# tatary/ramses

Measured on AMD Instinct MI355X. Metric: cell-updates/s (Godunov sweep), uniform Sedov3D, higher is better.
Workload: dtype f64

## Files before the change

ramses_amd/csrc/hydro_sweep.hip:

```cpp
#include <hip/hip_runtime.h>

#include <type_traits>

#include "difmag_core.hpp"
#include "hydro_core.hpp"
#include "sweep_args.hpp"

namespace ramses_amd {

#ifdef RAMSES_AMD_FAST
#define SWEEP_NS fastmode
#else
#define SWEEP_NS strictmode
#endif

namespace SWEEP_NS {

constexpr int BX = 64;
#ifndef TILE_SWEEP_BY
#define TILE_SWEEP_BY 12
#endif

template <int BY, int NV>
struct Plane {
  double v[NV][BY][BX];
};

template <int ST, int BY, int NV, bool MASK, bool GRAV, int NX = 0, bool DUTY = false, bool R3 = false, int DPN = 0>
struct Lds {
  static constexpr int NF = NV + NX;
  static constexpr int RING = (ST == 3 || R3) ? 3 : 2;
#ifndef SWEEP_PARK_PLAIN
#ifdef RAMSES_AMD_FAST
#define SWEEP_PARK_PLAIN 1
#else
#define SWEEP_PARK_PLAIN 0
#endif
#endif
  static constexpr bool PARK = MASK || ((GRAV || SWEEP_PARK_PLAIN) && BY == 12);
  static constexpr int MR = PARK ? BY - 2 : BY;
  static constexpr int M0 = PARK ? 1 : 0;
  static constexpr size_t q_off = 0;
  static constexpr size_t m_off = q_off + RING * sizeof(Plane<BY, NV>);
  static constexpr size_t park_off = m_off + 2 * sizeof(Plane<MR, NF>);
  static constexpr size_t duty_off = park_off + (PARK ? sizeof(double) * 2 * NF * (BY - 4) * BX : 0);
  static constexpr size_t mask_off = duty_off + (DUTY ? sizeof(double) * 2 * NF * BX : 0);
  static constexpr size_t sloc_off = mask_off + (MASK ? 3 * BY * BX : 0);
  static constexpr size_t dpark_off = sloc_off + (MASK ? 4 * BY * BX : 0);
  static constexpr size_t bytes = dpark_off + sizeof(double) * DPN * (BY - 4) * BX;
};
template <int RS, int NV>
constexpr int dif_parked() { return (NV == 5 && RS == RIEMANN_EXACT) ? 2 * NV + 2 : ((NV == 6) ? NV + 2 : 0); }

__device__ __forceinline__ double wave_shr1(double v) {
  int lo = __double2loint(v), hi = __double2hiint(v);
  lo = __builtin_amdgcn_update_dpp(lo, lo, 0x138, 0xf, 0xf, false);
  hi = __builtin_amdgcn_update_dpp(hi, hi, 0x138, 0xf, 0xf, false);
  return __hiloint2double(hi, lo);
}
template <bool TIED = false>
__device__ __forceinline__ double wave_shl1(double v) {
  int lo = __double2loint(v), hi = __double2hiint(v);
  lo = TIED ? __builtin_amdgcn_update_dpp(lo, lo, 0x130, 0xf, 0xf, false) : __builtin_amdgcn_update_dpp(0, lo, 0x130, 0xf, 0xf, true);
  hi = TIED ? __builtin_amdgcn_update_dpp(hi, hi, 0x130, 0xf, 0xf, false) : __builtin_amdgcn_update_dpp(0, hi, 0x130, 0xf, 0xf, true);
  return __hiloint2double(hi, lo);
}

enum { ROLE_HALO = 0, ROLE_LOW = 1, ROLE_HIGH = 2, ROLE_FULL = 3, ROLE_HALO_HI = 4, ROLE_FULL_LO = 5 };

#ifndef SWEEP_YDUTY
#define SWEEP_YDUTY 0
#endif
template <int ST, int RS, int BY, bool GRAV, int SCHEME, int NV, bool MASK, int NE = 0, bool PFIX = false>
constexpr bool y_duty() {
  return SWEEP_YDUTY && SWEEP_PARK_PLAIN && RS == RIEMANN_LLF && BY == 12 && ST != 3 && !GRAV && SCHEME == 0 && NV == 5 && !MASK && NE == 0 && !PFIX;
}
template <int BY, bool DUTY>
constexpr int yflux_wave(int f) { return !DUTY ? f : (f == 2 ? 0 : (f == BY - 2 ? BY - 1 : f)); }

#ifndef SWEEP_TRIM
#ifdef RAMSES_AMD_FAST
#define SWEEP_TRIM 1
#else
#define SWEEP_TRIM 0
#endif
#endif

#ifndef SWEEP_CYCLE_PROBE
#define SWEEP_CYCLE_PROBE 0
#endif
#if SWEEP_CYCLE_PROBE
constexpr int PROBE_BLOCKS = 8192, PROBE_ROWS = 12, PROBE_WORDS = 6;
static __device__ unsigned long long sweep_cycle_probe[PROBE_BLOCKS][PROBE_ROWS][PROBE_WORDS];
#endif

typedef unsigned int v2u32 __attribute__((ext_vector_type(2)));
constexpr unsigned BUF_RANGE = 0x7fffffffu;
constexpr unsigned BUF_OOB = 0xffffffffu;
#ifndef SWEEP_STORE_AUX
#define SWEEP_STORE_AUX 0
#endif
__device__ __forceinline__ double plane_load(const double *var_base, unsigned plane_bytes, unsigned off) {
  __amdgpu_buffer_rsrc_t r = __builtin_amdgcn_make_buffer_rsrc(const_cast<double *>(var_base), 0, BUF_RANGE, 0x00020000);
  return __builtin_bit_cast(double, __builtin_amdgcn_raw_buffer_load_b64(r, off, plane_bytes, 0));
}
__device__ __forceinline__ void plane_store(double *var_base, unsigned plane_bytes, unsigned off, double x) {
  __amdgpu_buffer_rsrc_t r = __builtin_amdgcn_make_buffer_rsrc(var_base, 0, BUF_RANGE, 0x00020000);
  __builtin_amdgcn_raw_buffer_store_b64(__builtin_bit_cast(v2u32, x), r, off, plane_bytes, SWEEP_STORE_AUX);
}

__device__ __forceinline__ int wave_shr1_i(int v) { return __builtin_amdgcn_update_dpp(v, v, 0x138, 0xf, 0xf, false); }
__device__ __forceinline__ int wave_shl1_i(int v) { return __builtin_amdgcn_update_dpp(0, v, 0x130, 0xf, 0xf, true); }
__device__ __forceinline__ int stat_load(const unsigned char *base, unsigned ncell, unsigned lane_cell, unsigned plane_cell) {
  __amdgpu_buffer_rsrc_t r = __builtin_amdgcn_make_buffer_rsrc(const_cast<unsigned char *>(base), 0, ncell, 0x00020000);
  return (int)__builtin_amdgcn_raw_buffer_load_b8(r, lane_cell, plane_cell, 0);
}
__device__ __forceinline__ int dir_load(const int *base, unsigned plane_ints, unsigned col) {
  __amdgpu_buffer_rsrc_t r = __builtin_amdgcn_make_buffer_rsrc(const_cast<int *>(base), 0, BUF_RANGE, 0x00020000);
  return (int)__builtin_amdgcn_raw_buffer_load_b32(r, col * 4u, plane_ints * 4u, 0);
}

template <int NV>
__device__ __forceinline__ void load_uold_cell(const double *uold, long pitch_var, unsigned odd_var, unsigned pb, unsigned off, double (&u)[NV]) {
#pragma unroll
  for (int n = 0; n < NV; n++) u[n] = plane_load(uold + (long)(n & ~1) * pitch_var, pb + (n & 1) * odd_var, off);
}
__device__ __forceinline__ unsigned tile_base_ym(int par, bool inB, unsigned a0, unsigned a1, unsigned b0, unsigned b1) {
  const unsigned a = par ? a1 : a0, b = par ? b1 : b0;
  return inB ? b : a;
}
template <int ST, int RS, int BY, bool GRAV, int SCHEME, int NV, int ROLE, bool MASK, int NE = 0, bool PFIX = false, bool DIFMAG = false>
__device__ __forceinline__ void sweep_march(const SweepArgs &A, unsigned char *smem_raw, const SweepPfix &X = SweepPfix(),
                                            const SweepDifmag &D = SweepDifmag()) {
  static_assert(!PFIX || (MASK && NE == 0 && SCHEME == 0), "pressure_fix: the sweep of a level in tiles, muscl");
  static_assert(!DIFMAG || (MASK && NE == 0 && SCHEME == 0 && !PFIX), "difmag: the sweep of a level in tiles, muscl, no pressure_fix");
  constexpr int NF = NV + (PFIX ? 2 : 0);
  const bool DXPOW2 = A.pow2 != 0;
  constexpr bool DUTY = y_duty<ST, RS, BY, GRAV, SCHEME, NV, MASK, NE, PFIX>();
  static_assert(DUTY || ROLE != ROLE_FULL_LO, "row 2 is a full row like the others unless the y fluxes are shared out");
  constexpr int DPN = DIFMAG ? dif_parked<RS, NV>() : 0;
  typedef Lds<ST, BY, NV, MASK, GRAV, NF - NV, DUTY, DIFMAG, DPN> L;
  double (*dpark)[BY - 4][BX] = reinterpret_cast<double (*)[BY - 4][BX]>(smem_raw + L::dpark_off);
  constexpr int RING = L::RING;
  constexpr bool PARK = L::PARK;
  constexpr int M0 = L::M0;
  Plane<BY, NV> *qring = reinterpret_cast<Plane<BY, NV> *>(smem_raw + L::q_off);
  Plane<L::MR, NF> *mring = reinterpret_cast<Plane<L::MR, NF> *>(smem_raw + L::m_off);
  double (*park)[BY - 4][BX] = reinterpret_cast<double (*)[BY - 4][BX]>(smem_raw + L::park_off);
  double (*yduty)[NF][BX] = reinterpret_cast<double (*)[NF][BX]>(smem_raw + L::duty_off);

  const int tx = threadIdx.x, ty = threadIdx.y;
  const HydroConst &P = A.P;

  const int hb = blockIdx.x;
  int bi = 0;
#pragma unroll
  for (int i = 1; i < 6; i++)
    if (i < A.nbox && hb >= A.box[i].first) bi = i;
  const SweepBox &B = A.box[bi];
  int lb = hb - B.first;
  {
    const int nxcd = 8;
    const int cnt = (bi + 1 < A.nbox ? A.box[bi + 1].first : (int)gridDim.x) - B.first;
    if (cnt % nxcd == 0) {
      const int per = cnt / nxcd;
      lb = (lb % nxcd) * per + lb / nxcd;
    }
  }
#ifndef SWEEP_TILE_YFAST
#define SWEEP_TILE_YFAST 0
#endif
#if SWEEP_TILE_YFAST
  const int tiy = B.ty0 + lb % B.nty;
  const int tix = B.tx0 + (lb / B.nty) % B.ntx;
#else
  const int tix = B.tx0 + lb % B.ntx;
  const int tiy = B.ty0 + (lb / B.ntx) % B.nty;
#endif
  const int tiz = lb / (B.ntx * B.nty);
  int x0 = tix * (BX - 4);
  int y0 = tiy * (BY - 4);
  int z0 = B.zlo + tiz * B.zchunk;
  int z1 = min(z0 + B.zchunk, B.zhi);
  if (MASK) {
    const int4 w = reinterpret_cast<const int4 *>(A.work)[hb];
    x0 = w.x; y0 = w.y; z0 = w.z; z1 = w.w;
  }

  const int xu = x0 - 2 + tx;
  const int yu = y0 - 2 + ty;
  int xi, yi;
  if (A.ng == 0) {
    xi = xu < 0 ? xu + A.nx : (xu >= A.nx ? xu - A.nx : xu);
    xi = xi >= A.nx ? xi % A.nx : xi;
    yi = yu < 0 ? yu + A.ny : (yu >= A.ny ? yu - A.ny : yu);
    yi = yi >= A.ny ? yi % A.ny : yi;
  } else {
    xi = min(max(xu, -A.ng), A.nx + A.ng - 1) + A.ng;
    yi = min(max(yu, -A.ng), A.ny + A.ng - 1) + A.ng;
  }
  const unsigned colb = (unsigned)(xi + yi * (int)A.pitch_y) * 8u;
  int tyu = 0, yis = 0, xa = 0, tA = 0, tB = 0, drow = 0;
  bool inB = false;
  unsigned *sloc = reinterpret_cast<unsigned *>(smem_raw + L::sloc_off);
  if (MASK) {
    tyu = __builtin_amdgcn_readfirstlane(ty);
    const int ys = y0 - 2 + tyu;
    yis = ys < 0 ? ys + A.ny : (ys >= A.ny ? ys - A.ny : ys);
    const int xs = x0 - 2;
    xa = xs < 0 ? xs + A.nx : xs;
    tA = xa >> 6; tB = tA + 1 < A.ntx ? tA + 1 : 0;
    inB = (xa & 63) + tx >= 64;
    drow = A.ntx * (yis >> 3);
    const int lind = (xi & 1) + 2 * (yis & 1);
    sloc[ty * BX + tx] = ((unsigned)((long)lind * A.ngd) + (unsigned)(((xi >> 1) & (TILE_OX - 1)) + TILE_OX * ((yis >> 1) & (TILE_OY - 1)))) * 8u;
  }
  const double *__restrict__ uold = A.uold;
  double *__restrict__ unew = A.unew;
  const double *__restrict__ grav = A.grav;

#ifndef SWEEP_LATE_BASE
#define SWEEP_LATE_BASE 0
#endif
  constexpr bool LATE = SWEEP_LATE_BASE && NV == 5;
#ifndef SWEEP_KEEP_PLAIN
#define SWEEP_KEEP_PLAIN 1
#endif
#ifndef SWEEP_KEEP_STRICT
#define SWEEP_KEEP_STRICT 0
#endif
#if defined(RAMSES_AMD_FAST) || SWEEP_KEEP_STRICT
#ifndef SWEEP_KEEP_LLF_ONLY
#define SWEEP_KEEP_LLF_ONLY 0
#endif
#ifndef SWEEP_KEEP_NOT_HLLC
#define SWEEP_KEEP_NOT_HLLC 1
#endif
  constexpr bool KEEP = (MASK || (SWEEP_KEEP_PLAIN && BY == 12)) && NV == 5 && !LATE && (!SWEEP_KEEP_LLF_ONLY || RS == RIEMANN_LLF) &&
                        (!SWEEP_KEEP_NOT_HLLC || RS != RIEMANN_HLLC);
#else
  constexpr bool KEEP = false;
#endif
  constexpr bool r_fxz = ROLE == ROLE_FULL || ROLE == ROLE_FULL_LO;
  constexpr bool r_trace = ROLE == ROLE_LOW || ROLE == ROLE_HIGH || r_fxz;
  constexpr bool y_give = DUTY && (ROLE == ROLE_FULL_LO || ROLE == ROLE_HIGH);
  constexpr bool y_take = DUTY && (ROLE == ROLE_HALO || ROLE == ROLE_HALO_HI);
  constexpr int DUTY_F = ROLE == ROLE_HALO ? 2 : BY - 2;
  static_assert(!DUTY || (yflux_wave<BY, DUTY>(2) == 0 && yflux_wave<BY, DUTY>(BY - 2) == BY - 1 && yflux_wave<BY, DUTY>(3) == 3),
                "the roles below implement this table");
  constexpr bool TRIM = SWEEP_TRIM != 0 && RS == RIEMANN_LLF && SCHEME == 0 && NE == 0 && !PFIX;
  const bool r_upd = r_fxz && (tx >= 2) && (tx <= BX - 3) && (xu < A.nx) && (yu < A.ny);
  const unsigned colb_upd = r_upd ? colb : BUF_OOB;

  const double dtdx = A.dt / A.dx;
  const double dtxhalf = A.dt * 0.5;

  auto plane_off = [&](int p) -> unsigned {
    int pz;
    if (A.ng == 0) { pz = p < 0 ? p + A.nz : (p >= A.nz ? p - A.nz : p); }
    else { pz = p + A.ng; }
    return (unsigned)pz * (unsigned)(A.pitch_z * 8);
  };
  auto wrap_z = [&](int p) -> int { return p < 0 ? p + A.nz : (p >= A.nz ? p - A.nz : p); };
  constexpr unsigned TILE_VOID = 0x80000000u;
  unsigned sA0 = TILE_VOID, sA1 = TILE_VOID, sB0 = TILE_VOID, sB1 = TILE_VOID;
  unsigned mA0 = TILE_VOID, mA1 = TILE_VOID, mB0 = TILE_VOID, mB1 = TILE_VOID;
  int drow_m = 0;
  if constexpr (DIFMAG) {
    const int ym = yis > 0 ? yis - 1 : A.ny - 1;
    drow_m = A.ntx * (ym >> 3);
  }
  auto tile_of_plane = [&](int p) -> int { return wrap_z(p) >> 3; };
  auto tile_set = [&](int tz) {
    typedef const int __attribute__((address_space(4))) *cdir_p;
    const cdir_p row = (cdir_p)(A.dir + (long)tz * (A.ntx * A.nty) + drow);
    const int ra = row[tA], rb = row[tB];
    const unsigned a = ra < 0 ? TILE_VOID : (unsigned)ra * 8u, b = rb < 0 ? TILE_VOID : (unsigned)rb * 8u;
    if (tz & 1) { sA1 = a; sB1 = b; } else { sA0 = a; sB0 = b; }
    if constexpr (DIFMAG) {
      const cdir_p rowm = (cdir_p)(A.dir + (long)tz * (A.ntx * A.nty) + drow_m);
      const int qa = rowm[tA], qb = rowm[tB];
      const unsigned am = qa < 0 ? TILE_VOID : (unsigned)qa * 8u, bm = qb < 0 ? TILE_VOID : (unsigned)qb * 8u;
      if (tz & 1) { mA1 = am; mB1 = bm; } else { mA0 = am; mB0 = bm; }
    }
  };
  auto zpart = [&](int p) -> unsigned {
    const int pz = wrap_z(p);
    return (unsigned)((long)(pz & 1) * 4 * A.ngd) + (unsigned)(TILE_OX * TILE_OY * ((pz >> 1) & (TILE_OZ - 1)));
  };
  auto tbp = [&](int p) -> unsigned {
    const int par = tile_of_plane(p) & 1;
    const unsigned a = par ? sA1 : sA0, b = par ? sB1 : sB0;
    return (inB ? b : a) + sloc[ty * BX + tx];
  };
  const unsigned odd_var = (unsigned)(A.pitch_var * 8);
  auto load_u = [&](int p, double (&u)[NV]) {
    const unsigned pb = MASK ? zpart(p) * 8u : plane_off(p), off = MASK ? tbp(p) : colb;
#pragma unroll
    for (int n = 0; n < NV; n++)
      u[n] = MASK ? plane_load(uold + (long)(n & ~1) * A.pitch_var, pb + (n & 1) * odd_var, off) : plane_load(uold + (long)n * A.pitch_var, pb, off);
  };
  const double *__restrict__ bsrc = A.base_uold ? uold : unew;
  auto load_base = [&](int p, double (&u)[NF]) {
    const unsigned pb = zpart(p) * 8u, off = tbp(p);
#pragma unroll
    for (int n = 0; n < NV; n++) u[n] = plane_load(bsrc + (long)(n & ~1) * A.pitch_var, pb + (n & 1) * odd_var, off);
    if constexpr (PFIX) { u[NV] = plane_load(X.divu, pb, off); u[NV + 1] = plane_load(X.enew, pb, off); }
  };
  double dif_cy = 0.0;
  double dif_c0 = 0.0, dif_c1 = 0.0;
  int ok_zlo = 0;
  int spre = 0;
  unsigned char *smask = smem_raw + L::mask_off;
  auto load_g = [&](int p, double (&g)[3]) {
    if (GRAV) {
      const unsigned pb = MASK ? zpart(p) * 8u : plane_off(p), off = MASK ? tbp(p) : colb;
#pragma unroll
      for (int d = 0; d < 3; d++) g[d] = plane_load(grav + (long)d * A.pitch_var, pb, off);
    } else {
      g[0] = g[1] = g[2] = 0.0;
    }
  };

  double qmz[NV];
  double fzlo[NF];
  double upre[NV], gpre[3];
  double rold = 0.0, sold[NV > 5 ? NV - 5 : 1];
  double ukeep[NV];
#pragma unroll
  for (int n = 0; n < NV; n++) ukeep[n] = 0.0;

  double rinv_c = 0.0;
#if SWEEP_CYCLE_PROBE
  unsigned long long pr_a = 0, pr_w = 0, pr_b = 0, pr_n = 0;
#endif

  int sa = 0, sb = 1, sc = 2;

  if (MASK) {
    const int t0 = tile_of_plane(z0 - 2), t1 = t0 + 1 < A.ntz ? t0 + 1 : 0;
    tile_set(t0);
    tile_set(t1);
    __syncthreads();
    if (r_trace) spre = stat_load(A.stat, (unsigned)A.pitch_var, tbp(z0 - 1) >> 3, zpart(z0 - 1));
  }
  {
    double u[NV], g[3], q[NV];
    load_u(z0 - 2, u); load_g(z0 - 2, g);
    ctoprim_cell<NV, GRAV, NE>(u, g, dtxhalf, P, q);
#pragma unroll
    for (int n = 0; n < NV; n++) qring[sa].v[n][ty][tx] = q[n];
    load_u(z0 - 1, u); load_g(z0 - 1, g);
    if (KEEP) {
#pragma unroll
      for (int n = 0; n < NV; n++) ukeep[n] = u[n];
    }
    if constexpr (TRIM && r_trace) ctoprim_cell<NV, GRAV, NE>(u, g, dtxhalf, P, q, &rinv_c);
    else ctoprim_cell<NV, GRAV, NE>(u, g, dtxhalf, P, q);
#pragma unroll
    for (int n = 0; n < NV; n++) qring[sb].v[n][ty][tx] = q[n];
    load_u(z0, upre); load_g(z0, gpre);
#pragma unroll
    for (int n = 0; n < NV; n++) qmz[n] = 1.0;
#pragma unroll
    for (int n = 0; n < NF; n++) fzlo[n] = 0.0;
  }
  __builtin_amdgcn_s_waitcnt(0x0f70);
  __syncthreads();

  const int txm = tx - 1, txp = tx + 1;
  const int tym = ty - 1, typ = ty + 1;

  double partx[NF];
  double fyown[NF];
  double rnew = 0.0, snew[NV > 5 ? NV - 5 : 1];
  double bcar[NV];
#pragma unroll
  for (int n = 0; n < NV; n++) bcar[n] = 0.0;
#pragma unroll
  for (int n = 0; n < NF; n++) { partx[n] = 0.0; fyown[n] = 0.0; }
  if (PARK && r_fxz) {
#pragma unroll
    for (int n = 0; n < 2 * NF; n++) park[n][ty - 2][tx] = 0.0;
  }
  if constexpr (DUTY && ROLE == ROLE_FULL_LO) {
#pragma unroll
    for (int n = 0; n < NF; n++) yduty[0][n][tx] = yduty[1][n][tx] = 0.0;
  }
  if constexpr (DPN > 0 && (ROLE == ROLE_FULL || ROLE == ROLE_FULL_LO)) {
#pragma unroll
    for (int n = 0; n < DPN; n++) dpark[n][ty - 2][tx] = n < NV + 2 ? 0.0 : 1.0;
  }

  for (int c = z0 - 1; c <= z1; c++) {
    Plane<L::MR, NF> &M = mring[c & 1];
    Plane<L::MR, NF> &Mprev = mring[(c & 1) ^ 1];
#if SWEEP_CYCLE_PROBE
    const unsigned long long pr_t0 = __builtin_readcyclecounter();
#endif
    double qc[NV];
    double rinv_n = 0.0;
    if constexpr (TRIM && r_trace) ctoprim_cell<NV, GRAV, NE>(upre, gpre, dtxhalf, P, qc, &rinv_n);
    else ctoprim_cell<NV, GRAV, NE>(upre, gpre, dtxhalf, P, qc);
    if (RING == 3 || !r_trace) {
#pragma unroll
      for (int n = 0; n < NV; n++) qring[RING == 3 ? sc : sa].v[n][ty][tx] = qc[n];
    }
    double ucur[NF];
    if (r_fxz && !LATE && !DIFMAG) {
      if (KEEP && (!MASK || A.base_uold)) {
#pragma unroll
        for (int n = 0; n < NV; n++) ucur[n] = ukeep[n];
      } else if constexpr (MASK) load_base(c, ucur);
      else load_u(c, ucur);
    }
    if (KEEP && r_fxz) {
#pragma unroll
      for (int n = 0; n < NV; n++) ukeep[n] = upre[n];
    }
    int okc = 0, ok_ym = 0;
    if (MASK && r_trace) {
      okc = spre;
      smask[((c + 3) % 3 * BY + ty) * BX + tx] = (unsigned char)okc;
    }

    double qpy[NV], dz[NF], px[NF];
    if (ST == 3) __syncthreads();
    if constexpr (r_trace) {
      const Plane<BY, NV> &qs = qring[sb];
      const Plane<BY, NV> &qprev = qring[sa];
      double qb[NV], dq[3][NV];
      if (ST == 3) {
        const Plane<BY, NV> &qnext = qring[sc];
        const int xs[3] = {txm, tx, txp}, ys[3] = {tym, ty, typ};
#pragma unroll
        for (int n = 0; n < NV; n++) {
          double nb[27], d3[3];
#pragma unroll
          for (int dj = 0; dj < 3; dj++)
#pragma unroll
            for (int di = 0; di < 3; di++) {
              nb[di + 3 * dj] = qprev.v[n][ys[dj]][xs[di]];
              nb[di + 3 * dj + 9] = qs.v[n][ys[dj]][xs[di]];
              nb[di + 3 * dj + 18] = qnext.v[n][ys[dj]][xs[di]];
            }
          qb[n] = nb[13];
          slope3_var(nb, d3);
          dq[0][n] = d3[0]; dq[1][n] = d3[1]; dq[2][n] = d3[2];
        }
      } else if (ST == 4 || ST == 5 || ST == 6) {
#pragma unroll
        for (int n = 0; n < NV; n++) qb[n] = qs.v[n][ty][tx];
        const double dc0 = qb[1] * A.dt / A.dx, dc1 = qb[2] * A.dt / A.dx, dc2 = qb[3] * A.dt / A.dx;
#pragma unroll
        for (int n = 0; n < NV; n++) {
          dq[0][n] = slope1_1d<ST>(qs.v[n][ty][txm], qb[n], qs.v[n][ty][txp], dc0, n);
          dq[1][n] = slope1_1d<ST>(qs.v[n][tym][tx], qb[n], qs.v[n][typ][tx], dc1, n);
          dq[2][n] = slope1_1d<ST>(qprev.v[n][ty][tx], qb[n], qc[n], dc2, n);
        }
      } else {
#pragma unroll
        for (int n = 0; n < NV; n++) {
          qb[n] = qs.v[n][ty][tx];
          dq[0][n] = slope1<ST>(qs.v[n][ty][txm], qb[n], qs.v[n][ty][txp], P);
          dq[1][n] = slope1<ST>(qs.v[n][tym][tx], qb[n], qs.v[n][typ][tx], P);
          dq[2][n] = slope1<ST>(qprev.v[n][ty][tx], qb[n], qc[n], P);
        }
      }
      if (RING == 2) {
#pragma unroll
        for (int n = 0; n < NV; n++) qring[sa].v[n][ty][tx] = qc[n];
      }
      double qm[3][NV], qp[3][NV];
      if (SCHEME == 0) {
        if constexpr (TRIM) trace3d_cell<NV, NE, r_fxz>(qb, dq, dtdx, dtdx, dtdx, P, qm, qp, &rinv_c);
        else trace3d_cell<NV, NE, r_fxz>(qb, dq, dtdx, dtdx, dtdx, P, qm, qp);
      } else {
        const double cc = ctoprim_sound(qb[0], qb[4], P);
        tracexyz_cell<NV>(qb, dq, cc, dtdx, dtdx, dtdx, P, qm, qp);
      }
#pragma unroll
      for (int n = 0; n < NV; n++) M.v[n][ty - M0][tx] = (DUTY && ROLE == ROLE_HIGH) ? qp[1][n] : qm[1][n];
#pragma unroll
      for (int n = 0; n < NV; n++) qpy[n] = qp[1][n];
      if constexpr (DUTY && ROLE == ROLE_FULL_LO) {
#pragma unroll
        for (int n = 0; n < NV; n++) yduty[c & 1][n][tx] = qp[1][n];
      }
      if constexpr (r_fxz) {
        double qL[NV], fx[NF], fz[NF];
#pragma unroll
        for (int n = 0; n < NV; n++) qL[n] = wave_shr1(qm[0][n]);
        if constexpr (PFIX) {
          double f[NV], t[2];
          scaled_interface_flux_tmp<RS, NV, 0>(qL, qp[0], P, A.dt, A.dx, A.rdx, DXPOW2, f, t);
#pragma unroll
          for (int n = 0; n < NV; n++) fx[n] = f[n];
          fx[NV] = t[0]; fx[NV + 1] = t[1];
          scaled_interface_flux_tmp<RS, NV, 2>(qmz, qp[2], P, A.dt, A.dx, A.rdx, DXPOW2, f, t);
#pragma unroll
          for (int n = 0; n < NV; n++) fz[n] = f[n];
          fz[NV] = t[0]; fz[NV + 1] = t[1];
        } else {
        scaled_interface_flux<RS, NV, 0, !MASK, NE, TRIM>(qL, qp[0], P, A.dt, A.dx, A.rdx, dtdx, DXPOW2, fx);
        if constexpr (DPN > NV + 2) {
#pragma unroll
          for (int n = 0; n < NV; n++) qmz[n] = dpark[NV + 2 + n][ty - 2][tx];
        }
        scaled_interface_flux<RS, NV, 2, !MASK, NE, TRIM>(qmz, qp[2], P, A.dt, A.dx, A.rdx, dtdx, DXPOW2, fz);
        }
        if (MASK && !DIFMAG) {
          const int s_xm = wave_shr1_i(okc);
          const bool zx = ((okc | s_xm) & CELL_REFINED) != 0, zz = ((okc | ok_zlo) & CELL_REFINED) != 0;
#pragma unroll
          for (int n = 0; n < NF; n++) { fx[n] = zx ? 0.0 : fx[n]; fz[n] = zz ? 0.0 : fz[n]; }
        }
        double fxh[NF];
#pragma unroll
        for (int n = 0; n < NV; n++) qmz[n] = qm[2][n];
        if constexpr (DPN > NV + 2) {
#pragma unroll
          for (int n = 0; n < NV; n++) dpark[NV + 2 + n][ty - 2][tx] = qm[2][n];
        }
        if constexpr (DIFMAG) {
#pragma unroll
          for (int n = 0; n < NF; n++) { px[n] = fx[n]; dz[n] = fz[n]; }
        } else {
#pragma unroll
        for (int n = 0; n < NF; n++) {
          dz[n] = fzlo[n] - fz[n];
          fzlo[n] = fz[n];
          fxh[n] = wave_shl1(fx[n]);
          px[n] = LATE ? (fx[n] - fxh[n]) : ucur[n] + (fx[n] - fxh[n]);
        }
        }
        if (NV > 5 + NE && !MASK) {
          rnew = ucur[0];
#pragma unroll
          for (int n = 5 + NE; n < NV; n++) snew[n - 5] = ucur[n];
        }
      }
    }
    __builtin_amdgcn_sched_barrier(0);
    if constexpr (DIFMAG && (r_fxz || ROLE == ROLE_HIGH)) {
      static_assert(!KEEP && !LATE && PARK, "difmag borrows ukeep, bcar and partx");
      double (&dif_u)[NV] = ukeep, (&dif_uym)[NV] = bcar, (&dif_uzm)[NV] = partx;
      load_uold_cell<NV>(uold, A.pitch_var, odd_var, zpart(c) * 8u, tbp(c), dif_u);
      if constexpr (!r_fxz)
        load_uold_cell<NV>(uold, A.pitch_var, odd_var, zpart(c) * 8u,
                           tile_base_ym(tile_of_plane(c) & 1, inB, mA0, mA1, mB0, mB1) + sloc[(ty - 1) * BX + tx], dif_uym);
      if constexpr (r_fxz) {
        load_uold_cell<NV>(uold, A.pitch_var, odd_var, zpart(c - 1) * 8u, tbp(c - 1), dif_uzm);
        load_base(c, ucur);
      }
    }
    {
      const int pn = min(c + 2, z1 + 1);
      if (MASK) {
        const int lp = wrap_z(pn) & 7;
        const int tn = tile_of_plane(pn) + 1 < A.ntz ? tile_of_plane(pn) + 1 : 0;
        if (lp == 4) tile_set(tn);
      }
      load_u(pn, upre); load_g(pn, gpre);
      if (MASK && r_trace) { const int ps = min(c + 1, z1 + 1); spre = stat_load(A.stat, (unsigned)A.pitch_var, tbp(ps) >> 3, zpart(ps)); }
    }
    __builtin_amdgcn_sched_barrier(0);
#if SWEEP_CYCLE_PROBE
    const unsigned long long pr_t1 = __builtin_readcyclecounter();
#endif
    __syncthreads();
#if SWEEP_CYCLE_PROBE
    const unsigned long long pr_t2 = __builtin_readcyclecounter();
#endif

    if constexpr (DIFMAG && (r_fxz || ROLE == ROLE_HIGH)) {
      double (&dif_u)[NV] = ukeep, (&dif_uym)[NV] = bcar, (&dif_uzm)[NV] = partx;
      const Plane<BY, NV> &q0 = qring[sb], &q1 = qring[sc];
      constexpr int NR = r_fxz ? 3 : 2;
      const double fdiv = 0.25 / A.dx;
      double dsum[3][2];
#pragma unroll
      for (int d = 0; d < 3; d++) {
        double vo[2][NR], vl[2][NR];
#pragma unroll
        for (int r = 0; r < NR; r++) {
          vo[0][r] = q0.v[1 + d][tym + r][tx];
          vo[1][r] = q1.v[1 + d][tym + r][tx];
          vl[0][r] = wave_shr1(vo[0][r]);
          vl[1][r] = wave_shr1(vo[1][r]);
        }
#pragma unroll
        for (int r0 = 0; r0 < NR - 1; r0++) {
          double v[2][2][2];
#pragma unroll
          for (int dk = 0; dk < 2; dk++)
#pragma unroll
            for (int dj = 0; dj < 2; dj++) { v[dk][dj][0] = vl[dk][r0 + dj]; v[dk][dj][1] = vo[dk][r0 + dj]; }
          dsum[d][r0] = d == 0 ? difmag::cmpdivu_ux(v, fdiv) : (d == 1 ? difmag::cmpdivu_vy(v, fdiv) : difmag::cmpdivu_wz(v, fdiv));
        }
        if (NR == 2) dsum[d][1] = 0.0;
      }
      const double dn[2] = {dsum[0][0] + dsum[1][0] + dsum[2][0], dsum[0][1] + dsum[1][1] + dsum[2][1]};
      if constexpr (DPN > 0 && r_fxz) {
        dif_c0 = dpark[NV][ty - 2][tx]; dif_c1 = dpark[NV + 1][ty - 2][tx];
#pragma unroll
        for (int n = 0; n < NV; n++) fzlo[n] = dpark[n][ty - 2][tx];
      }
      const double c0x = wave_shl1<true>(dif_c0), n0x = wave_shl1<true>(dn[0]);
      dif_cy = difmag::consup_coef(D.difmag, difmag::consup_div1_y(dif_c0, c0x, dn[0], n0x));
      if constexpr (r_fxz) {
        const double c1x = wave_shl1<true>(dif_c1);
        const double cx = difmag::consup_coef(D.difmag, difmag::consup_div1_x(dif_c0, dif_c1, dn[0], dn[1]));
        const double cz = difmag::consup_coef(D.difmag, difmag::consup_div1_z(dif_c0, c0x, dif_c1, c1x));
        const int s_xm = wave_shr1_i(okc);
        const bool zx = ((okc | s_xm) & CELL_REFINED) != 0, zz = ((okc | ok_zlo) & CELL_REFINED) != 0;
#pragma unroll
        for (int n = 0; n < NV; n++) {
          const double fxd = difmag::consup_term(px[n], A.dt, cx, dif_u[n], wave_shr1(dif_u[n]));
          const double fzd = difmag::consup_term(dz[n], A.dt, cz, dif_u[n], dif_uzm[n]);
          const double fxn = zx ? 0.0 : fxd, fzn = zz ? 0.0 : fzd;
          dz[n] = fzlo[n] - fzn;
          fzlo[n] = fzn;
          px[n] = ucur[n] + (fxn - wave_shl1<true>(fxn));
        }
      }
      dif_c0 = dn[0]; dif_c1 = dn[1];
      if constexpr (DPN > 0 && r_fxz) {
        dpark[NV][ty - 2][tx] = dn[0]; dpark[NV + 1][ty - 2][tx] = dn[1];
#pragma unroll
        for (int n = 0; n < NV; n++) dpark[n][ty - 2][tx] = fzlo[n];
      }
      if constexpr (r_fxz)
        load_uold_cell<NV>(uold, A.pitch_var, odd_var, zpart(c) * 8u,
                           tile_base_ym(tile_of_plane(c) & 1, inB, mA0, mA1, mB0, mB1) + sloc[(ty - 1) * BX + tx], dif_uym);
    }
    double fy[NF];
    if constexpr (y_take) {
      double qL[NV], qR[NV];
#pragma unroll
      for (int n = 0; n < NV; n++) {
        qL[n] = M.v[n][DUTY_F - 1 - M0][tx];
        qR[n] = ROLE == ROLE_HALO ? yduty[c & 1][n][tx] : M.v[n][DUTY_F - M0][tx];
      }
      scaled_interface_flux<RS, NV, 1, !MASK, NE, TRIM>(qL, qR, P, A.dt, A.dx, A.rdx, dtdx, DXPOW2, fy);
#pragma unroll
      for (int n = 0; n < NF; n++) {
        if (ROLE == ROLE_HALO) yduty[c & 1][n][tx] = fy[n];
        else M.v[n][DUTY_F - 1 - M0][tx] = fy[n];
      }
    }
    if constexpr ((r_fxz || ROLE == ROLE_HIGH) && !y_give) {
      double qL[NV];
#pragma unroll
      for (int n = 0; n < NV; n++) qL[n] = M.v[n][tym - M0][tx];
      if constexpr (PFIX) {
        double f[NV], t[2];
        scaled_interface_flux_tmp<RS, NV, 1>(qL, qpy, P, A.dt, A.dx, A.rdx, DXPOW2, f, t);
#pragma unroll
        for (int n = 0; n < NV; n++) fy[n] = f[n];
        fy[NV] = t[0]; fy[NV + 1] = t[1];
      } else {
      scaled_interface_flux<RS, NV, 1, !MASK, NE, TRIM>(qL, qpy, P, A.dt, A.dx, A.rdx, dtdx, DXPOW2, fy);
      }
      if constexpr (DIFMAG) {
        double (&dif_u)[NV] = ukeep, (&dif_uym)[NV] = bcar;
#pragma unroll
        for (int n = 0; n < NV; n++) fy[n] = difmag::consup_term(fy[n], A.dt, dif_cy, dif_u[n], dif_uym[n]);
      }
      if (MASK) {
        ok_ym = smask[((c + 3) % 3 * BY + tym) * BX + tx];
        const bool zy = ((okc | ok_ym) & CELL_REFINED) != 0;
#pragma unroll
        for (int n = 0; n < NF; n++) fy[n] = zy ? 0.0 : fy[n];
      }
#pragma unroll
      for (int n = 0; n < NF; n++) M.v[n][tym - M0][tx] = fy[n];
    }
    if constexpr (r_fxz) {
      double un[NF], fyh[NF];
#pragma unroll
      for (int n = 0; n < NF; n++) {
        fyh[n] = Mprev.v[n][ty - M0][tx];
        const double pxn = PARK ? park[n][ty - 2][tx] : partx[n];
        const double fyn = y_give ? yduty[(c & 1) ^ 1][n][tx] : (PARK ? park[NF + n][ty - 2][tx] : fyown[n]);
        const double part = (LATE ? bcar[n < NV ? n : 0] + pxn : pxn) + (fyn - fyh[n]);
        un[n] = part + dz[n];
      }
      if (NV > 5 + NE && !MASK) {
        if (rold < P.smallr && un[0] > rold) {
#pragma unroll
          for (int n = 5 + NE; n < NV; n++) un[n] = sold[n - 5] * dmaxd(un[0], P.smallr) / P.smallr;
        } else if (un[0] < P.smallr && rold > un[0]) {
#pragma unroll
          for (int n = 5 + NE; n < NV; n++) un[n] = sold[n - 5] * P.smallr / dmaxd(rold, P.smallr);
        }
        rold = rnew;
#pragma unroll
        for (int n = 5 + NE; n < NV; n++) sold[n - 5] = snew[n - 5];
      }
#pragma unroll
      for (int n = 0; n < NF; n++) {
        if (PARK) { park[n][ty - 2][tx] = px[n]; if (!y_give) park[NF + n][ty - 2][tx] = fy[n]; }
        else { partx[n] = px[n]; fyown[n] = fy[n]; }
      }
      {
        const unsigned pb = MASK ? zpart(c - 1) * 8u : plane_off(c - 1);
        const unsigned so = (c >= z0 + 1) ? (MASK ? ((r_upd && (ok_zlo & CELL_OWNED)) ? tbp(c - 1) : BUF_OOB) : colb_upd) : BUF_OOB;
#pragma unroll
        for (int n = 0; n < NV; n++) {
          if (MASK) plane_store(unew + (long)(n & ~1) * A.pitch_var, pb + (n & 1) * odd_var, so, un[n]);
          else plane_store(unew + (long)n * A.pitch_var, pb, so, un[n]);
        }
        if constexpr (PFIX) { plane_store(X.divu, pb, so, un[NV]); plane_store(X.enew, pb, so, un[NV + 1]); }
      }
      if constexpr (LATE) { if (MASK) load_base(c, bcar); else load_u(c, bcar); }
    }
    if (RING == 3) { const int t = sa; sa = sb; sb = sc; sc = t; }
    else { const int t = sa; sa = sb; sb = t; }
    if (MASK) ok_zlo = okc;
    if (TRIM) rinv_c = rinv_n;
#if SWEEP_CYCLE_PROBE
    pr_a += pr_t1 - pr_t0; pr_w += pr_t2 - pr_t1; pr_b += __builtin_readcyclecounter() - pr_t2; pr_n += 1;
#endif
  }
#if SWEEP_CYCLE_PROBE
  if (tx == 0 && blockIdx.x < PROBE_BLOCKS && ty < PROBE_ROWS) {
    unsigned long long *o = sweep_cycle_probe[blockIdx.x][ty];
    o[0] = pr_a; o[1] = pr_w; o[2] = pr_b; o[3] = pr_n; o[4] = (unsigned long long)ty;
    o[5] = (unsigned long long)__builtin_amdgcn_s_getreg((31 << 11) | 4);
  }
#endif
}

template <int ST, int RS, int BY, bool GRAV, int SCHEME, int NV, bool MASK = false>
__global__ __launch_bounds__(BX *BY) void godunov_sweep_kernel(SweepArgs A) {
  extern __shared__ __attribute__((aligned(16))) unsigned char smem_raw[];
  const int ty = threadIdx.y;
  if (ty >= 2 && ty <= BY - 3) __builtin_amdgcn_s_setprio(3);
  if (ty == 0) sweep_march<ST, RS, BY, GRAV, SCHEME, NV, ROLE_HALO, MASK>(A, smem_raw);
  else if (ty == BY - 1) sweep_march<ST, RS, BY, GRAV, SCHEME, NV, ROLE_HALO_HI, MASK>(A, smem_raw);
  else if (ty == 1) sweep_march<ST, RS, BY, GRAV, SCHEME, NV, ROLE_LOW, MASK>(A, smem_raw);
  else if (ty == BY - 2) sweep_march<ST, RS, BY, GRAV, SCHEME, NV, ROLE_HIGH, MASK>(A, smem_raw);
  else {
    if constexpr (y_duty<ST, RS, BY, GRAV, SCHEME, NV, MASK>()) {
      if (ty == 2) { sweep_march<ST, RS, BY, GRAV, SCHEME, NV, ROLE_FULL_LO, MASK>(A, smem_raw); return; }
    }
    sweep_march<ST, RS, BY, GRAV, SCHEME, NV, ROLE_FULL, MASK>(A, smem_raw);
  }
}

#ifndef RAMSES_AMD_FAST
template <int ST, int NV>
struct PfixRows {
  static constexpr int BY = (ST == 3 && NV == 7) ? 6 : 8;
};
template <int ST, int RS, int BY, bool GRAV, int NV>
__global__ __launch_bounds__(BX *BY) void godunov_sweep_pfix_kernel(SweepArgs A, SweepPfix X) {
  extern __shared__ __attribute__((aligned(16))) unsigned char smem_raw[];
  static_assert(Lds<ST, BY, NV, true, GRAV, 2>::bytes <= 160 * 1024, "the pressure_fix sweep fits one workgroup's LDS");
  const int ty = threadIdx.y;
  if (ty >= 2 && ty <= BY - 3) __builtin_amdgcn_s_setprio(3);
  if (ty == 0) sweep_march<ST, RS, BY, GRAV, 0, NV, ROLE_HALO, true, 0, true>(A, smem_raw, X);
  else if (ty == BY - 1) sweep_march<ST, RS, BY, GRAV, 0, NV, ROLE_HALO_HI, true, 0, true>(A, smem_raw, X);
  else if (ty == 1) sweep_march<ST, RS, BY, GRAV, 0, NV, ROLE_LOW, true, 0, true>(A, smem_raw, X);
  else if (ty == BY - 2) sweep_march<ST, RS, BY, GRAV, 0, NV, ROLE_HIGH, true, 0, true>(A, smem_raw, X);
  else sweep_march<ST, RS, BY, GRAV, 0, NV, ROLE_FULL, true, 0, true>(A, smem_raw, X);
}
#endif

#ifndef RAMSES_AMD_FAST
template <int ST, int RS, int BY, bool GRAV, int NV>
__global__ __launch_bounds__(BX *BY) void godunov_sweep_difmag_kernel(SweepArgs A, SweepDifmag D) {
  extern __shared__ __attribute__((aligned(16))) unsigned char smem_raw[];
  static_assert(Lds<ST, BY, NV, true, GRAV, 0, false, true, dif_parked<RS, NV>()>::bytes <= 160 * 1024, "the difmag sweep fits one workgroup's LDS");
  const int ty = threadIdx.y;
  if (ty >= 2 && ty <= BY - 3) __builtin_amdgcn_s_setprio(3);
  if (ty == 0) sweep_march<ST, RS, BY, GRAV, 0, NV, ROLE_HALO, true, 0, false, true>(A, smem_raw, SweepPfix(), D);
  else if (ty == BY - 1) sweep_march<ST, RS, BY, GRAV, 0, NV, ROLE_HALO_HI, true, 0, false, true>(A, smem_raw, SweepPfix(), D);
  else if (ty == 1) sweep_march<ST, RS, BY, GRAV, 0, NV, ROLE_LOW, true, 0, false, true>(A, smem_raw, SweepPfix(), D);
  else if (ty == BY - 2) sweep_march<ST, RS, BY, GRAV, 0, NV, ROLE_HIGH, true, 0, false, true>(A, smem_raw, SweepPfix(), D);
  else sweep_march<ST, RS, BY, GRAV, 0, NV, ROLE_FULL, true, 0, false, true>(A, smem_raw, SweepPfix(), D);
}
#endif

template <int ST, int RS, int NV, int NE>
__global__ __launch_bounds__(BX * 8) void godunov_sweep_nener_kernel(SweepArgs A) {
  extern __shared__ __attribute__((aligned(16))) unsigned char smem_raw[];
  constexpr int BY = 8;
  const int ty = threadIdx.y;
  if (ty >= 2 && ty <= BY - 3) __builtin_amdgcn_s_setprio(3);
  if (ty == 0) sweep_march<ST, RS, BY, false, 0, NV, ROLE_HALO, false, NE>(A, smem_raw);
  else if (ty == BY - 1) sweep_march<ST, RS, BY, false, 0, NV, ROLE_HALO_HI, false, NE>(A, smem_raw);
  else if (ty == 1) sweep_march<ST, RS, BY, false, 0, NV, ROLE_LOW, false, NE>(A, smem_raw);
  else if (ty == BY - 2) sweep_march<ST, RS, BY, false, 0, NV, ROLE_HIGH, false, NE>(A, smem_raw);
  else sweep_march<ST, RS, BY, false, 0, NV, ROLE_FULL, false, NE>(A, smem_raw);
}

// ... 581 lines not shown
    return launch_surface(surface_flux_difmag_kernel<ST, decltype(r)::value, decltype(nv)::value, decltype(g)::value>, s, A, D);
  });
}
#endif

static int plan_boxes(SweepArgs &A, int by) {
  const int NTX = (A.nx + (BX - 4) - 1) / (BX - 4);
  const int NTY = (A.ny + (by - 4) - 1) / (by - 4);
  const int zb = 2;
  const bool splittable = NTX >= 3 && NTY >= 3 && A.nz >= 4 * zb;
  A.nbox = 0;
  int nblocks = 0;
  auto add_box = [&](int tx0, int tx1, int ty0, int ty1, int zlo, int zhi, int zchunk) {
    if (tx1 <= tx0 || ty1 <= ty0 || zhi <= zlo) return;
    SweepBox &B = A.box[A.nbox++];
    B.tx0 = tx0; B.ntx = tx1 - tx0; B.ty0 = ty0; B.nty = ty1 - ty0;
    B.zlo = zlo; B.zhi = zhi; B.zchunk = zchunk < (zhi - zlo) ? zchunk : (zhi - zlo);
    B.first = nblocks;
    nblocks += B.ntx * B.nty * ((zhi - zlo + B.zchunk - 1) / B.zchunk);
  };
  const int zc = A.zchunk;
  if (A.region == SWEEP_ALL || (A.region == SWEEP_SHELL && !splittable)) {
    add_box(0, NTX, 0, NTY, 0, A.nz, zc);
  } else if (A.region == SWEEP_INTERIOR) {
    if (splittable) add_box(1, NTX - 1, 1, NTY - 1, zb, A.nz - zb, zc);
  } else if (A.region == SWEEP_SHELL) {
    const int zs = 32;
    add_box(0, 1, 1, NTY - 1, zb, A.nz - zb, zs);
    add_box(NTX - 1, NTX, 1, NTY - 1, zb, A.nz - zb, zs);
    add_box(0, NTX, 0, 1, zb, A.nz - zb, zs);
    add_box(0, NTX, NTY - 1, NTY, zb, A.nz - zb, zs);
    add_box(0, NTX, 0, NTY, 0, zb, zs);
    add_box(0, NTX, 0, NTY, A.nz - zb, A.nz, zs);
  } else {
    return -1;
  }
  if (nblocks == 0) return 0;
  A.nblocks = nblocks;
  return nblocks;
}

static bool tile_items(SweepArgs &A) {
  if (!A.stat || !A.dir || !A.work || A.ng != 0 || A.nwork <= 0) return false;
  A.nblocks = A.nwork;
  A.nbox = 1;
  return true;
}

template <int ST, int RS, int BY, bool GRAV, int SCHEME, int NV, bool MASK>
static hipError_t launch_sweep(const SweepArgs &A, hipStream_t s) {
  if constexpr (!sweep_variant(ST, RS, BY, GRAV, SCHEME, NV, MASK)) {
    return hipErrorInvalidValue;
  } else {
    typedef Lds<ST, BY, NV, MASK, GRAV, 0, y_duty<ST, RS, BY, GRAV, SCHEME, NV, MASK>()> L;
    static_assert(L::bytes <= 160 * 1024, "one workgroup's LDS");
    return launch_kernel(godunov_sweep_kernel<ST, RS, BY, GRAV, SCHEME, NV, MASK>, dim3(A.nblocks), dim3(BX, BY), L::bytes, s, A);
  }
}
template <int ST>
hipError_t SweepOf<ST>::sweep(SweepArgs &A, int rs, int by, int scheme, int nvar, bool grav, hipStream_t s) {
  return pick(rs, Solvers(), [&](auto r) {
    constexpr int RS = decltype(r)::value;
    const bool tiles = A.stat != nullptr;
    const int rows = sweep_rows(ST, RS, nvar, scheme, tiles);
    if (by == 0 || rows == 8) by = rows;
    const int planned = plan_boxes(A, by);
    if (planned < 0) return hipErrorInvalidValue;
    if (planned == 0) return hipSuccess;
    if (tiles) {
      if (!tile_items(A)) return hipErrorInvalidValue;
    } else if (!is_1d(ST) && nvar == 5 && scheme != 1) {
      scheme = 0;
    }
    return pick(by, IntList<8, 12, TILE_SWEEP_BY>(), [&](auto b) { return pick(nvar, Nvars(), [&](auto nv) { return pick(scheme, Schemes(), [&](auto sc) {
      return pick(grav, [&](auto g) { return pick(tiles, [&](auto m) {
        return launch_sweep<ST, RS, decltype(b)::value, decltype(g)::value, decltype(sc)::value, decltype(nv)::value, decltype(m)::value>(A, s);
      }); }); }); }); });
  });
}

#ifndef RAMSES_AMD_FAST
template <int ST>
hipError_t SweepOf<ST>::pfix(SweepArgs &A, const SweepPfix &X, int rs, int nvar, bool grav, hipStream_t s) {
  if (!X.divu || !X.enew || !tile_items(A)) return hipErrorInvalidValue;
  A.box[0] = SweepBox{0, 1, 0, 1, 0, A.nz, A.nz, 0};
  return pick_variant(SolversOf<ST>(), rs, nvar, grav, [&](auto r, auto nv, auto g) {
    constexpr int RS = decltype(r)::value, NV = decltype(nv)::value, BY = PfixRows<ST, NV>::BY;
    constexpr bool GRAV = decltype(g)::value;
    return launch_kernel(godunov_sweep_pfix_kernel<ST, RS, BY, GRAV, NV>, dim3(A.nblocks), dim3(BX, BY), Lds<ST, BY, NV, true, GRAV, 2>::bytes, s, A, X);
  });
}
template <int ST>
hipError_t SweepOf<ST>::difmag(SweepArgs &A, const SweepDifmag &D, int rs, int nvar, bool grav, hipStream_t s) {
  if (!(D.difmag > 0.0) || !tile_items(A)) return hipErrorInvalidValue;
  A.box[0] = SweepBox{0, 1, 0, 1, 0, A.nz, A.nz, 0};
  return pick_variant(SolversOf<ST>(), rs, nvar, grav, [&](auto r, auto nv, auto g) {
    constexpr int RS = decltype(r)::value, NV = decltype(nv)::value, BY = 8;
    constexpr bool GRAV = decltype(g)::value;
    return launch_kernel(godunov_sweep_difmag_kernel<ST, RS, BY, GRAV, NV>, dim3(A.nblocks), dim3(BX, BY),
                         Lds<ST, BY, NV, true, GRAV, 0, false, true, dif_parked<RS, NV>()>::bytes, s, A, D);
  });
}
#endif

template <int ST>
hipError_t SweepOf<ST>::nener(SweepArgs &A, int rs, int nvar, int nener, hipStream_t s) {
  return pick(rs, SolversOf<ST>(), [&](auto r) {
// ... 147 lines not shown
```

Measured before the change: 45.86 billion.

## Add per-phase wave priority ladder and split y-duty into hi-only mode

Replaces the static priority boost for interior rows with a per-phase ladder of s_setprio marks (top, traced, x-flux, fluxes, barrier) chosen per role and kernel family. The aim is to steer the wave scheduler so that the critical-path rows reach the barrier sooner and reduce barrier stall time. It also adds a y-duty mode where only the high halo row takes over a y flux, with a temporary priority raise for that taker. The cycle probe is expanded to seven spans. Priority changes can starve other waves and may help or hurt depending on the kernel family.

```diff
diff --git a/ramses_amd/csrc/hydro_sweep.hip b/ramses_amd/csrc/hydro_sweep.hip
--- a/ramses_amd/csrc/hydro_sweep.hip
+++ b/ramses_amd/csrc/hydro_sweep.hip
@@ -75,8 +75,55 @@
 constexpr bool y_duty() {
   return SWEEP_YDUTY && SWEEP_PARK_PLAIN && RS == RIEMANN_LLF && BY == 12 && ST != 3 && !GRAV && SCHEME == 0 && NV == 5 && !MASK && NE == 0 && !PFIX;
 }
-template <int BY, bool DUTY>
-constexpr int yflux_wave(int f) { return !DUTY ? f : (f == 2 ? 0 : (f == BY - 2 ? BY - 1 : f)); }
+template <int ST, int RS, int BY, bool GRAV, int SCHEME, int NV, bool MASK, int NE = 0, bool PFIX = false>
+constexpr bool y_duty_lo() { return SWEEP_YDUTY == 1 && y_duty<ST, RS, BY, GRAV, SCHEME, NV, MASK, NE, PFIX>(); }
+template <int BY, bool DUTY, bool DUTY_LO>
+constexpr int yflux_wave(int f) { return !DUTY ? f : ((DUTY_LO && f == 2) ? 0 : (f == BY - 2 ? BY - 1 : f)); }
+
+#ifndef SWEEP_PRIO_LADDER
+#define SWEEP_PRIO_LADDER 1
+#endif
+#ifndef SWEEP_PRIO_FAMILIES
+#define SWEEP_PRIO_FAMILIES 30
+#endif
+enum { MARK_BARRIER = 0, MARK_TOP = 1, MARK_TRACED = 2, MARK_XFLUX = 3, MARK_FLUXES = 4, MARK_COUNT = 5 };
+template <int ST, int RS, int BY, bool GRAV, int SCHEME, int NV, bool MASK, int NE = 0, bool PFIX = false, bool DIFMAG = false>
+constexpr bool prio_ladder() {
+#ifdef RAMSES_AMD_FAST
+  constexpr bool fast = true;
+#else
+  constexpr bool fast = false;
+#endif
+  if (!SWEEP_PRIO_LADDER || ST == 3 || SCHEME != 0 || NE != 0 || PFIX || DIFMAG) return false;
+  const int family = (fast && RS == RIEMANN_LLF) ? 1 : (MASK ? 16 : (BY != 12 ? 8 : (!fast ? 4 : 2)));
+  return (SWEEP_PRIO_FAMILIES & family) != 0;
+}
+constexpr int prio_of(int role, int mark) {
+  const bool full = role == ROLE_FULL || role == ROLE_FULL_LO;
+#if SWEEP_PRIO_LADDER == 2
+  if (full) return mark == MARK_BARRIER ? 3 : (mark == MARK_TRACED ? 2 : (mark == MARK_FLUXES ? 1 : -1));
+  if (role == ROLE_HIGH || role == ROLE_LOW) return mark == MARK_BARRIER ? 1 : -1;
+#elif SWEEP_PRIO_LADDER == 3
+  if (full) return mark == MARK_BARRIER ? 3 : (mark == MARK_TRACED ? 2 : (mark == MARK_XFLUX ? 1 : (mark == MARK_FLUXES ? 0 : -1)));
+  if (role == ROLE_HIGH || role == ROLE_LOW) return mark == MARK_BARRIER ? 1 : -1;
+#elif SWEEP_PRIO_LADDER == 4
+  if (full) return mark == MARK_BARRIER ? 3 : (mark == MARK_TOP ? 2 : (mark == MARK_TRACED ? 1 : -1));
+  if (role == ROLE_HIGH) return mark == MARK_BARRIER ? 0 : (mark == MARK_TOP ? 1 : -1);
+  if (role == ROLE_LOW) return mark == MARK_BARRIER ? 1 : -1;
+#elif SWEEP_PRIO_LADDER == 5
+  if (full) return mark == MARK_BARRIER ? 3 : (mark == MARK_TRACED ? 2 : (mark == MARK_FLUXES ? 1 : -1));
+  if (role == ROLE_HIGH || role == ROLE_LOW) return mark == MARK_BARRIER ? 2 : -1;
+#else
+  if (full) return mark == MARK_BARRIER ? 3 : (mark == MARK_TRACED ? 2 : (mark == MARK_FLUXES ? 1 : -1));
+  if (role == ROLE_HIGH) return mark == MARK_BARRIER ? 1 : (mark == MARK_TOP ? 2 : -1);
+  if (role == ROLE_LOW) return mark == MARK_BARRIER ? 1 : -1;
+#endif
+  return -1;
+}
+template <bool LADDER, int ROLE, int MARK>
+__device__ __forceinline__ void prio_mark() {
+  if constexpr (LADDER && prio_of(ROLE, MARK) >= 0) __builtin_amdgcn_s_setprio(prio_of(ROLE, MARK));
+}
 
 #ifndef SWEEP_TRIM
 #ifdef RAMSES_AMD_FAST
@@ -90,7 +137,8 @@
 #define SWEEP_CYCLE_PROBE 0
 #endif
 #if SWEEP_CYCLE_PROBE
-constexpr int PROBE_BLOCKS = 8192, PROBE_ROWS = 12, PROBE_WORDS = 6;
+constexpr int PROBE_BLOCKS = 8192, PROBE_ROWS = 12, PROBE_SPANS = 7, PROBE_WORDS = PROBE_SPANS + 3;
+#define SWEEP_PROBE_NOW(t) do { __builtin_amdgcn_sched_barrier(0); (t) = __builtin_readcyclecounter(); __builtin_amdgcn_sched_barrier(0); } while (0)
 static __device__ unsigned long long sweep_cycle_probe[PROBE_BLOCKS][PROBE_ROWS][PROBE_WORDS];
 #endif
 
@@ -137,9 +185,11 @@
   constexpr int NF = NV + (PFIX ? 2 : 0);
   const bool DXPOW2 = A.pow2 != 0;
   constexpr bool DUTY = y_duty<ST, RS, BY, GRAV, SCHEME, NV, MASK, NE, PFIX>();
-  static_assert(DUTY || ROLE != ROLE_FULL_LO, "row 2 is a full row like the others unless the y fluxes are shared out");
+  constexpr bool DUTY_LO = y_duty_lo<ST, RS, BY, GRAV, SCHEME, NV, MASK, NE, PFIX>();
+  static_assert(DUTY_LO || ROLE != ROLE_FULL_LO, "row 2 is a full row like the others unless its -y face is handed over");
+  constexpr bool LADDER = prio_ladder<ST, RS, BY, GRAV, SCHEME, NV, MASK, NE, PFIX, DIFMAG>();
   constexpr int DPN = DIFMAG ? dif_parked<RS, NV>() : 0;
-  typedef Lds<ST, BY, NV, MASK, GRAV, NF - NV, DUTY, DIFMAG, DPN> L;
+  typedef Lds<ST, BY, NV, MASK, GRAV, NF - NV, DUTY_LO, DIFMAG, DPN> L;
   double (*dpark)[BY - 4][BX] = reinterpret_cast<double (*)[BY - 4][BX]>(smem_raw + L::dpark_off);
   constexpr int RING = L::RING;
   constexpr bool PARK = L::PARK;
@@ -244,10 +294,12 @@
   constexpr bool r_fxz = ROLE == ROLE_FULL || ROLE == ROLE_FULL_LO;
   constexpr bool r_trace = ROLE == ROLE_LOW || ROLE == ROLE_HIGH || r_fxz;
   constexpr bool y_give = DUTY && (ROLE == ROLE_FULL_LO || ROLE == ROLE_HIGH);
-  constexpr bool y_take = DUTY && (ROLE == ROLE_HALO || ROLE == ROLE_HALO_HI);
+  constexpr bool y_take = DUTY && ((DUTY_LO && ROLE == ROLE_HALO) || ROLE == ROLE_HALO_HI);
   constexpr int DUTY_F = ROLE == ROLE_HALO ? 2 : BY - 2;
-  static_assert(!DUTY || (yflux_wave<BY, DUTY>(2) == 0 && yflux_wave<BY, DUTY>(BY - 2) == BY - 1 && yflux_wave<BY, DUTY>(3) == 3),
+  static_assert(!DUTY || (yflux_wave<BY, DUTY, DUTY_LO>(2) == (DUTY_LO ? 0 : 2) && yflux_wave<BY, DUTY, DUTY_LO>(BY - 2) == BY - 1 &&
+                          yflux_wave<BY, DUTY, DUTY_LO>(3) == 3),
                 "the roles below implement this table");
+  constexpr bool take_prio = y_take && !DUTY_LO;
   constexpr bool TRIM = SWEEP_TRIM != 0 && RS == RIEMANN_LLF && SCHEME == 0 && NE == 0 && !PFIX;
   const bool r_upd = r_fxz && (tx >= 2) && (tx <= BX - 3) && (xu < A.nx) && (yu < A.ny);
   const unsigned colb_upd = r_upd ? colb : BUF_OOB;
@@ -332,7 +384,7 @@
 
   double rinv_c = 0.0;
 #if SWEEP_CYCLE_PROBE
-  unsigned long long pr_a = 0, pr_w = 0, pr_b = 0, pr_n = 0;
+  unsigned long long pr_s[PROBE_SPANS] = {0, 0, 0, 0, 0, 0, 0}, pr_n = 0;
 #endif
 
   int sa = 0, sb = 1, sc = 2;
@@ -396,8 +448,10 @@
     Plane<L::MR, NF> &M = mring[c & 1];
     Plane<L::MR, NF> &Mprev = mring[(c & 1) ^ 1];
 #if SWEEP_CYCLE_PROBE
-    const unsigned long long pr_t0 = __builtin_readcyclecounter();
-#endif
+    unsigned long long pr_t0, pr_ts = 0, pr_t1, pr_t2, pr_ty = 0, pr_tf = 0, pr_tw = 0, pr_te;
+    SWEEP_PROBE_NOW(pr_t0);
+#endif
+    prio_mark<LADDER, ROLE, MARK_TOP>();
     double qc[NV];
     double rinv_n = 0.0;
     if constexpr (TRIM && r_trace) ctoprim_cell<NV, GRAV, NE>(upre, gpre, dtxhalf, P, qc, &rinv_n);
@@ -471,6 +525,9 @@
 #pragma unroll
         for (int n = 0; n < NV; n++) qring[sa].v[n][ty][tx] = qc[n];
       }
+#if SWEEP_CYCLE_PROBE
+      SWEEP_PROBE_NOW(pr_ts);
+#endif
       double qm[3][NV], qp[3][NV];
       if (SCHEME == 0) {
         if constexpr (TRIM) trace3d_cell<NV, NE, r_fxz>(qb, dq, dtdx, dtdx, dtdx, P, qm, qp, &rinv_c);
@@ -487,6 +544,7 @@
 #pragma unroll
         for (int n = 0; n < NV; n++) yduty[c & 1][n][tx] = qp[1][n];
       }
+      prio_mark<LADDER, ROLE, MARK_TRACED>();
       if constexpr (r_fxz) {
         double qL[NV], fx[NF], fz[NF];
 #pragma unroll
@@ -503,6 +561,7 @@
           fz[NV] = t[0]; fz[NV + 1] = t[1];
         } else {
         scaled_interface_flux<RS, NV, 0, !MASK, NE, TRIM>(qL, qp[0], P, A.dt, A.dx, A.rdx, dtdx, DXPOW2, fx);
+        prio_mark<LADDER, ROLE, MARK_XFLUX>();
         if constexpr (DPN > NV + 2) {
 #pragma unroll
           for (int n = 0; n < NV; n++) qmz[n] = dpark[NV + 2 + n][ty - 2][tx];
@@ -542,6 +601,7 @@
       }
     }
     __builtin_amdgcn_sched_barrier(0);
+    prio_mark<LADDER, ROLE, MARK_FLUXES>();
     if constexpr (DIFMAG && (r_fxz || ROLE == ROLE_HIGH)) {
       static_assert(!KEEP && !LATE && PARK, "difmag borrows ukeep, bcar and partx");
       double (&dif_u)[NV] = ukeep, (&dif_uym)[NV] = bcar, (&dif_uzm)[NV] = partx;
@@ -566,12 +626,14 @@
     }
     __builtin_amdgcn_sched_barrier(0);
 #if SWEEP_CYCLE_PROBE
-    const unsigned long long pr_t1 = __builtin_readcyclecounter();
+    SWEEP_PROBE_NOW(pr_t1);
 #endif
     __syncthreads();
 #if SWEEP_CYCLE_PROBE
-    const unsigned long long pr_t2 = __builtin_readcyclecounter();
-#endif
+    SWEEP_PROBE_NOW(pr_t2);
+#endif
+    prio_mark<LADDER, ROLE, MARK_BARRIER>();
+    if constexpr (take_prio) __builtin_amdgcn_s_setprio(3);
 
     if constexpr (DIFMAG && (r_fxz || ROLE == ROLE_HIGH)) {
       double (&dif_u)[NV] = ukeep, (&dif_uym)[NV] = bcar, (&dif_uzm)[NV] = partx;
@@ -642,17 +704,27 @@
         qL[n] = M.v[n][DUTY_F - 1 - M0][tx];
         qR[n] = ROLE == ROLE_HALO ? yduty[c & 1][n][tx] : M.v[n][DUTY_F - M0][tx];
       }
+#if SWEEP_CYCLE_PROBE
+      SWEEP_PROBE_NOW(pr_ty);
+#endif
       scaled_interface_flux<RS, NV, 1, !MASK, NE, TRIM>(qL, qR, P, A.dt, A.dx, A.rdx, dtdx, DXPOW2, fy);
 #pragma unroll
       for (int n = 0; n < NF; n++) {
         if (ROLE == ROLE_HALO) yduty[c & 1][n][tx] = fy[n];
         else M.v[n][DUTY_F - 1 - M0][tx] = fy[n];
       }
+      if constexpr (take_prio) __builtin_amdgcn_s_setprio(0);
+#if SWEEP_CYCLE_PROBE
+      SWEEP_PROBE_NOW(pr_tf);
+#endif
     }
     if constexpr ((r_fxz || ROLE == ROLE_HIGH) && !y_give) {
       double qL[NV];
 #pragma unroll
       for (int n = 0; n < NV; n++) qL[n] = M.v[n][tym - M0][tx];
+#if SWEEP_CYCLE_PROBE
+      SWEEP_PROBE_NOW(pr_ty);
+#endif
       if constexpr (PFIX) {
         double f[NV], t[2];
         scaled_interface_flux_tmp<RS, NV, 1>(qL, qpy, P, A.dt, A.dx, A.rdx, DXPOW2, f, t);
@@ -675,6 +747,9 @@
       }
 #pragma unroll
       for (int n = 0; n < NF; n++) M.v[n][tym - M0][tx] = fy[n];
+#if SWEEP_CYCLE_PROBE
+      SWEEP_PROBE_NOW(pr_tf);
+#endif
     }
     if constexpr (r_fxz) {
       double un[NF], fyh[NF];
@@ -713,6 +788,9 @@
         }
         if constexpr (PFIX) { plane_store(X.divu, pb, so, un[NV]); plane_store(X.enew, pb, so, un[NV + 1]); }
       }
+#if SWEEP_CYCLE_PROBE
+      SWEEP_PROBE_NOW(pr_tw);
+#endif
       if constexpr (LATE) { if (MASK) load_base(c, bcar); else load_u(c, bcar); }
     }
     if (RING == 3) { const int t = sa; sa = sb; sb = sc; sc = t; }
@@ -720,14 +798,22 @@
     if (MASK) ok_zlo = okc;
     if (TRIM) rinv_c = rinv_n;
 #if SWEEP_CYCLE_PROBE
-    pr_a += pr_t1 - pr_t0; pr_w += pr_t2 - pr_t1; pr_b += __builtin_readcyclecounter() - pr_t2; pr_n += 1;
+    SWEEP_PROBE_NOW(pr_te);
+    if (!pr_ts) pr_ts = pr_t0;
+    if (!pr_ty) pr_ty = pr_t2;
+    if (!pr_tf) pr_tf = pr_ty;
+    if (!pr_tw) pr_tw = pr_tf;
+    pr_s[0] += pr_ts - pr_t0; pr_s[1] += pr_t1 - pr_ts; pr_s[2] += pr_t2 - pr_t1; pr_s[3] += pr_ty - pr_t2;
+    pr_s[4] += pr_tf - pr_ty; pr_s[5] += pr_tw - pr_tf; pr_s[6] += pr_te - pr_tw; pr_n += 1;
 #endif
   }
 #if SWEEP_CYCLE_PROBE
   if (tx == 0 && blockIdx.x < PROBE_BLOCKS && ty < PROBE_ROWS) {
     unsigned long long *o = sweep_cycle_probe[blockIdx.x][ty];
-    o[0] = pr_a; o[1] = pr_w; o[2] = pr_b; o[3] = pr_n; o[4] = (unsigned long long)ty;
-    o[5] = (unsigned long long)__builtin_amdgcn_s_getreg((31 << 11) | 4);
+#pragma unroll
+    for (int k = 0; k < PROBE_SPANS; k++) o[k] = pr_s[k];
+    o[PROBE_SPANS] = pr_n; o[PROBE_SPANS + 1] = (unsigned long long)ty;
+    o[PROBE_SPANS + 2] = (unsigned long long)__builtin_amdgcn_s_getreg((31 << 11) | 4);
   }
 #endif
 }
@@ -736,13 +822,15 @@
 __global__ __launch_bounds__(BX *BY) void godunov_sweep_kernel(SweepArgs A) {
   extern __shared__ __attribute__((aligned(16))) unsigned char smem_raw[];
   const int ty = threadIdx.y;
-  if (ty >= 2 && ty <= BY - 3) __builtin_amdgcn_s_setprio(3);
+  if constexpr (!prio_ladder<ST, RS, BY, GRAV, SCHEME, NV, MASK>()) {
+    if (ty >= 2 && ty <= BY - 3) __builtin_amdgcn_s_setprio(3);
+  }
   if (ty == 0) sweep_march<ST, RS, BY, GRAV, SCHEME, NV, ROLE_HALO, MASK>(A, smem_raw);
   else if (ty == BY - 1) sweep_march<ST, RS, BY, GRAV, SCHEME, NV, ROLE_HALO_HI, MASK>(A, smem_raw);
   else if (ty == 1) sweep_march<ST, RS, BY, GRAV, SCHEME, NV, ROLE_LOW, MASK>(A, smem_raw);
   else if (ty == BY - 2) sweep_march<ST, RS, BY, GRAV, SCHEME, NV, ROLE_HIGH, MASK>(A, smem_raw);
   else {
-    if constexpr (y_duty<ST, RS, BY, GRAV, SCHEME, NV, MASK>()) {
+    if constexpr (y_duty_lo<ST, RS, BY, GRAV, SCHEME, NV, MASK>()) {
       if (ty == 2) { sweep_march<ST, RS, BY, GRAV, SCHEME, NV, ROLE_FULL_LO, MASK>(A, smem_raw); return; }
     }
     sweep_march<ST, RS, BY, GRAV, SCHEME, NV, ROLE_FULL, MASK>(A, smem_raw);
@@ -1430,7 +1518,7 @@
   if constexpr (!sweep_variant(ST, RS, BY, GRAV, SCHEME, NV, MASK)) {
     return hipErrorInvalidValue;
   } else {
-    typedef Lds<ST, BY, NV, MASK, GRAV, 0, y_duty<ST, RS, BY, GRAV, SCHEME, NV, MASK>()> L;
+    typedef Lds<ST, BY, NV, MASK, GRAV, 0, y_duty_lo<ST, RS, BY, GRAV, SCHEME, NV, MASK>()> L;
     static_assert(L::bytes <= 160 * 1024, "one workgroup's LDS");
     return launch_kernel(godunov_sweep_kernel<ST, RS, BY, GRAV, SCHEME, NV, MASK>, dim3(A.nblocks), dim3(BX, BY), L::bytes, s, A);
   }
```

Result: no change. 45.86 billion (median of 2 runs) (+0.0%).
